# IDLabMedia/image-lens-reproject

Measured on AMD Instinct MI355X. Metric: Mpix/s reprojected (4K RGBA float, bicubic), higher is better.
Workload: dtype f32; 1 GPU; fisheye_to_rect_bicubic: 4096x4096x4 f32 -> 4096x4096x4, eqd->rect, interp=2, num_samples=1; frames_per_launch=16, parallelism=image-sharded x1 (static blocks of the sorted list), no collective

## Files before the change

### image-lens-reproject_amd/csrc/lrp_win_kernel.h

```cpp
#pragma once

#include "lrp_kernel_common.h"
#include "lrp_corner_fill.h"
#include "lrp_tile_kernel.h"
#include "lrp_win_plan.h"
#include "lrp_win_tiers.h"

namespace lrp {

#if defined(LRP_WAVE_STAMPS)
__device__ unsigned long long g_wave_stamps[3 * 65536];
#endif
#if defined(LRP_TIER_STATS)
__device__ unsigned g_tier_stats[8];
#endif


template <int OutLens, int InMode, int QMode, int CH, bool Frames = false, bool GeoRead = false, bool SS = false>
#ifndef LRP_WIN_MINWAVES5
#define LRP_WIN_MINWAVES5 3
#endif
#ifndef LRP_WIN_MINWAVES_AXIS
#define LRP_WIN_MINWAVES_AXIS 4
#endif
#ifndef LRP_WIN_MINWAVES_RAYS
#define LRP_WIN_MINWAVES_RAYS 3
#endif
#ifndef LRP_WIN_MINWAVES_FRAMES
#define LRP_WIN_MINWAVES_FRAMES 4
#endif
#ifndef LRP_WIN_CAP_BIG
#define LRP_WIN_CAP_BIG 1120
#endif
#ifndef LRP_WIN_CAP_BIG5
#define LRP_WIN_CAP_BIG5 1200
#endif
#ifndef LRP_WIN_MINWAVES_BIG
#define LRP_WIN_MINWAVES_BIG 2
#endif
__global__ __launch_bounds__(kWinThreads, (GeoRead && OutLens == kEquirect) ? LRP_WIN_MINWAVES_BIG : CH == 5 ? LRP_WIN_MINWAVES5 : (QMode == 4 ? LRP_WIN_MINWAVES_RAYS : (Frames ? LRP_WIN_MINWAVES_FRAMES : (QMode >= 2 ? LRP_WIN_MINWAVES_AXIS : LRP_WIN_MINWAVES)))) void reproject_bicubic_win_kernel(const KParams Pk) {
  constexpr bool Quad = QMode != 0;
  constexpr bool MirX = QMode == 1 || QMode == 3 || QMode == 4, MirY = QMode == 1 || QMode == 2 || QMode == 4;
  constexpr bool kSharedRays = QMode == 4;
  static_assert(QMode != 4 || OutLens == kEquidistant, "shared rays: the equidistant target");
  constexpr int kAllMirrors = (MirX ? 1 : 0) | (MirY ? 2 : 0);
  using WinBlock = WinBlockT<Quad>;
  static_assert(CH == 3 || CH == 4 || CH == 5, "window kernel: RGB, RGBA or RGBAZ");
  static_assert(!SS || (QMode == 0 && !Frames), "supersampling: plain blocks, no frame loop");
  constexpr int kBlockRows = SS ? 4 : kBlkH;
  static_assert(QMode != 2 || (OutLens != kEquidistant && InMode != kInEquidistant), "rows-only mirroring goes through the column-separable source x");
  static_assert(QMode != 3 || OutLens == kRect, "columns-only mirroring needs vz == -1");
  static_assert(!GeoRead || (QMode == 0 && (OutLens == kRect || (OutLens == kEquirect && !Frames))),
                "GeoRead: plain blocks, one instantiation per source mode (+ the big-window variants)");
  constexpr bool kBigWin = GeoRead && OutLens == kEquirect;
  constexpr int kCap = kBigWin ? (CH == 5 ? LRP_WIN_CAP_BIG5 : LRP_WIN_CAP_BIG) : kWinCap;
#ifndef LRP_BIG_PASSCOLS
#define LRP_BIG_PASSCOLS 64
#endif
  constexpr int kMaxPassCols = kBigWin ? LRP_BIG_PASSCOLS : 64;
  constexpr bool kGeoWrite = !GeoRead && !Frames && QMode == 0 && kWinWaves == 1;
  const bool geo_write = kGeoWrite && (Pk.geo_mode == 1 || Pk.geo_mode == 3) && blockIdx.y == 0;
  const int frames_per_wave = Frames ? (Pk.frames_per_wave > 0 ? Pk.frames_per_wave : 1) : 1;
  const int frame0 = Pk.batch_n > 0 ? (int)blockIdx.y * frames_per_wave : 0;
  const int n_frames = (Frames && Pk.batch_n > 0) ? min(frames_per_wave, Pk.batch_n - frame0) : 1;
  auto frame_src = [&](int f) { return Pk.batch_n > 0 ? Pk.batch_src[frame0 + f] : Pk.src; };
  auto frame_dst = [&](int f) { return Pk.batch_n > 0 ? Pk.batch_dst[frame0 + f] : Pk.dst; };
  KParams P = Pk;
  P.src = frame_src(0);
  P.dst = frame_dst(0);
  constexpr bool kOneBlock = Frames && GeoRead;
  constexpr bool Loop = (InMode == kInEquirectLoop);
  constexpr bool kEdge = InMode == kInRect;
#ifndef LRP_BIG_MAXCOLS
#define LRP_BIG_MAXCOLS 64
#endif
  constexpr bool kSplit = !Frames && (InMode == kInEquirect || InMode == kInEquirectLoop || (InMode == kInRect && CH == 5) || kBigWin);
  constexpr int kMaxStagedCols = kBigWin ? LRP_BIG_MAXCOLS : 64;
  constexpr bool kPassWin = (kSplit || (GeoRead && OutLens == kEquirect)) && (OutLens == kRect || GeoRead || (InMode == kInRect && CH == 5));
  constexpr bool kCoefHere = !kBigWin;
  constexpr bool kTapDma = kBigWin && kWinWaves == 1;
  constexpr int kOutSlots = (CH == 5 && kTapDma) ? 80 : 0;
  static_assert(!kTapDma || (CH == 5 ? (kCap + kOutSlots) * 16 >= 1024 * 20 : kCap >= 1024), "tap DMA: 16 taps x 64 pixels");
  constexpr bool kTapRotate = CH == 5 || kCap < 1027;
  __shared__ float4 s_win[kWinWaves][kCap + kOutSlots];
#ifndef LRP_BIG_PASS_SLOTS
#define LRP_BIG_PASS_SLOTS 4096
#endif
  constexpr int kPassCap = (kTapDma && LRP_BIG_PASS_SLOTS < kCap) ? LRP_BIG_PASS_SLOTS : kCap;

  constexpr bool kListable = GeoRead && InMode == kInRect;
  auto fill_share = [&]() {
    if constexpr (kListable) {
      const uint32_t per_wave = Pk.geo_fill_per_wave;
      if (per_wave != 0 && blockIdx.x % Pk.geo_fill_stride == 0) {
        const uint32_t total = Pk.geo_n_runs * 16u, s0 = blockIdx.x / Pk.geo_fill_stride * per_wave;
        if (s0 < total)
          for (int f = 0; f < n_frames; ++f) corner_fill_rows<CH, kOneBlock>(Pk, frame_src(f), frame_dst(f), s0, min(s0 + per_wave, total));
      }
    }
  };
  int tx, ty;
  bool listed = false;
  constexpr bool kListRec = kListable && kBigWin;
  int list_rec[7] = {0, 0, 0, 0, 0, 0, 0};
  bool have_list_rec = false;
  if constexpr (kListable) listed = Pk.geo_work != nullptr;
  if (listed) {
    typedef const int32_t __attribute__((address_space(4))) *ScalarI;
    const uintptr_t base = reinterpret_cast<uintptr_t>(Pk.geo_work);
    const uint64_t addr = ((uint64_t)(uint32_t)__builtin_amdgcn_readfirstlane((int)(uint32_t)(base >> 32)) << 32 |
                           (uint32_t)__builtin_amdgcn_readfirstlane((int)(uint32_t)base)) + (uint64_t)blockIdx.x * 8u;
    const ScalarI e = reinterpret_cast<ScalarI>(addr);
    tx = e[0];
    ty = e[1];
    if (kListRec && Pk.geo_work_rec != nullptr) {
      const uintptr_t rbase = reinterpret_cast<uintptr_t>(Pk.geo_work_rec);
      const ScalarI r = reinterpret_cast<ScalarI>(((uint64_t)(uint32_t)__builtin_amdgcn_readfirstlane((int)(uint32_t)(rbase >> 32)) << 32 |
                                                   (uint32_t)__builtin_amdgcn_readfirstlane((int)(uint32_t)rbase)) + (uint64_t)blockIdx.x * 32u);
#pragma unroll
      for (int i = 0; i < 7; ++i) list_rec[i] = r[i];
      have_list_rec = true;
    }
    if (tx < 0) {
      fill_share();
      return;
    }
  } else if (!xcd_tile<kWinXcdBand>(P.tiles_x, P.tiles_y, tx, ty, blockIdx.x)) return;
#if defined(LRP_WAVE_STAMPS)
  const unsigned long long stamp_start = wall_clock64();
#endif
  constexpr bool kAliasPairs = (OutLens == kEquirect || GeoRead) && InMode == kInRect && kWinWaves == 1;
  int g_flip = 0;
  bool g_reverse = false;
  if (kAliasPairs && P.alias_pairs != 0 && !listed) {
    if constexpr (QMode == 1) {
      g_flip = (tx & 1) ? 3 : 0;
      tx = (tx & 1) ? P.tiles_x - 1 - (tx >> 1) : (tx >> 1);
    } else if constexpr (QMode == 2) {
      if ((P.tiles_x & 1) == 0) {
        g_flip = (tx & 1) ? 2 : 0;
        tx = (tx >> 1) + ((tx & 1) ? P.tiles_x >> 1 : 0);
      }
    } else if ((P.tiles_x & 1) == 0) {
      g_reverse = (tx & 1) != 0;
      tx = (tx >> 1) + (g_reverse ? P.tiles_x >> 1 : 0);
      ty = g_reverse ? P.tiles_y - 1 - ty : ty;
    }
  }
  int lane = (int)(threadIdx.x & 63u);
  const int wave = __builtin_amdgcn_readfirstlane((int)(threadIdx.x >> 6));
  const int Gs = kOneBlock ? 1 : P.blocks_per_wave;
  const int G = kOneBlock ? 1 : GeoRead ? min(Gs, (P.y_end - P.y_offset + kBlockRows - 1) / kBlockRows - ty * Gs) : Gs;
  auto block_row = [&](int g) { return kOneBlock ? 0 : (kAliasPairs && g_reverse) ? G - 1 - g : g; };
  auto geo_classes = [&]() { return reinterpret_cast<uint8_t *>(P.geo_box) + geo_class_offset(P.out_w, P.out_h); };
  auto geo_class_index = [&](int g) { return (uint32_t)tx * geo_block_rows(P.out_h) + (uint32_t)(ty * Gs + block_row(g)); };
  auto geo_block = [&](int g) { return (uint32_t)(ty * Gs + block_row(g)) * (uint32_t)P.tiles_x + (uint32_t)tx; };
  constexpr bool quad = Quad;
  const int qw = MirX ? (P.out_w + 1) >> 1 : P.out_w;
  const int qh = MirY ? (P.out_h + 1) >> 1 : P.y_end;
  auto image_of = [&](int g) { return ((QMode == 2 ? 2 * g : g) ^ g_flip) & (QMode == 2 ? kAllMirrors : -1); };
  int prow, pcol;
  win_lane_pixel(lane, prow, pcol);
  const int ss_ns = SS ? Pk.num_samples : 1, ss_n = ss_ns * ss_ns, ss_npx = SS ? 64 / ss_n : kBlkW;
  int ss_x = 0, ss_y = 0;
  bool ss_owner = false;
  if constexpr (SS) {
    const int l = min(lane, ss_npx * ss_n - 1);
    pcol = ss_n == 4 ? l >> 2 : ss_n == 16 ? l >> 4 : (l * 57) >> 9;
    prow = 0;
    const int sub = l - pcol * ss_n;
    ss_x = ss_ns == 2 ? sub >> 1 : ss_ns == 4 ? sub >> 2 : (sub * 11) >> 5;
    ss_y = sub - ss_x * ss_ns;
    ss_owner = sub == ss_n - 1 && lane < ss_npx * ss_n;
  }
  const int x = tx * ((SS ? ss_npx : kBlkW) * kWinWaves) + wave * (SS ? ss_npx : kBlkW) + pcol;
  const int y_lane = P.y_offset + ty * (quad ? kBlkH : kBlockRows * Gs) + prow;
  auto pixel_row = [&](int g, int k) { return y_lane + (quad ? 0 : kBlockRows * block_row(g)) + (SS ? k : kPassRows * k); };
  const int xe = x < qw ? x : qw - 1;
  const int in_w = P.in_w;
  SrcView src = source_view<2, CH>(P);
  auto set_frame = [&](int f) {
    P.src = frame_src(f);
    P.dst = frame_dst(f);
    src = source_view<2, CH>(P);
  };
  float4 *const win0 = s_win[wave];
  constexpr bool kRunsEverywhere = CH == 5 && (OutLens == kEquirect || GeoRead) && InMode == kInRect;
  float *out_lds = nullptr;
  if constexpr (CH == 5 && kOutSlots != 0) {
    out_lds = reinterpret_cast<float *>(win0 + kCap);
  } else if constexpr (CH == 5) {
    __shared__ __attribute__((aligned(16))) float s_out[kWinWaves][320];
    out_lds = s_out[wave];
  }
  ColTerms col{0.0f, 0.0f, 0.0f, 0.0f, 0.0f};
  if constexpr (!GeoRead) col = column_terms<OutLens>(P, xe, ss_x);
  ColTerms col_m = col;
  if constexpr (MirX && !kSharedRays) col_m = column_terms<OutLens>(P, P.out_w - 1 - xe, 0);
  float qa[4] = {0.0f, 0.0f, 0.0f, 0.0f}, qb[4] = {0.0f, 0.0f, 0.0f, 0.0f};
  constexpr bool kInEqr = InMode == kInEquirect || InMode == kInEquirectLoop;
  constexpr bool kEqrByTheta = QMode == 3 && kInEqr;
  float qc[(kEqrByTheta || kSharedRays) ? 4 : 1] = {};
  auto quad_xy = [&](int g, int k, float &sx, float &sy) {
    const bool mx = (g & 1) != 0, my = (g >> 1) != 0;
    if constexpr (kSharedRays) {
      const int yk = y_lane + kPassRows * k;
      const uint32_t sgn_x = (mx && 2 * xe != P.out_w - 1) ? 0x80000000u : 0u;
      const uint32_t sgn_y = (my && 2 * yk != P.out_h - 1) ? 0x80000000u : 0u;
      float u, v;
      ray_to_plane<InMode>(P, u2f(f2u(qa[k]) ^ sgn_x), u2f(f2u(qb[k]) ^ sgn_y), qc[k], u, v);
      plane_to_texel<OutLens, InMode>(P, col, u, v, sx, sy);
    } else if constexpr (kEqrByTheta) {
      sx = mx ? qc[k] : qa[k];
      sy = qb[k];
    } else if constexpr (kInEqr) {
      sx = mx ? col_m.sx : col.sx;
      sy = my ? qb[k] : qa[k];
    } else {
      const uint32_t sgn_x = mx ? 0x80000000u : 0u, sgn_y = my ? 0x80000000u : 0u;
      plane_to_texel<OutLens, InMode>(P, mx ? col_m : col, u2f(f2u(qa[k]) ^ sgn_x), u2f(f2u(qb[k]) ^ sgn_y), sx, sy);
    }
  };

  const WinPlanLimits plan_limits = win_plan_limits(P);
  auto slots_of_rows = [](int pitch, int rows) { return win_slots_of_rows<CH>(pitch, rows); };
  auto raw_slots = [&](const WinBlock &b) { return win_raw_slots<CH, kSplit>(b); };
  auto plan_window = [&](WinBlock &b, int w_lo_x, int w_hi_x, int w_lo_ya, int w_hi_ya, int w_lo_yb, int w_hi_yb, bool exact_x, bool exact_y) {
    win_plan_block<CH, Loop, kSplit, kEdge, kCap, kMaxStagedCols>(b, P, plan_limits, w_lo_x, w_hi_x, w_lo_ya, w_hi_ya, w_lo_yb, w_hi_yb, exact_x, exact_y);
  };
  auto clear_block = [](WinBlock &b) { win_clear_block(b); };
  struct Extremes {
// ... 259 lines not shown
      const uint32_t first_row = (uint32_t)__builtin_amdgcn_readfirstlane((int)((uint32_t)b.y_lo * src.row_bytes));
      const uint32_t first_col = (uint32_t)__builtin_amdgcn_readfirstlane((int)((uint32_t)b.x_lo * (4u * CH)));
      const char *first = reinterpret_cast<const char *>(frame) + ((size_t)first_row + (size_t)first_col);
      const uint32_t lds0 = (uint32_t)(uintptr_t)(__attribute__((address_space(3))) void *)win0;
      for (int c0 = 0; c0 < n; c0 += 64) {
        if (c0 + lane < n) {
          const uint32_t lane_bytes = (uint32_t)(c0 + lane) * step;
          const uint32_t lds = lds0 + (uint32_t)c0 * 16u;
          if constexpr (CH == 3)
            asm volatile("s_mov_b32 m0, %0\n\ts_nop 0\n\tglobal_load_lds_dwordx3 %1, %2"
                         :
                         : "s"(__builtin_amdgcn_readfirstlane(lds)), "v"(lane_bytes), "s"(first)
                         : "memory", "m0");
          else
            asm volatile("s_mov_b32 m0, %0\n\ts_nop 0\n\tglobal_load_lds_dwordx4 %1, %2"
                         :
                         : "s"(__builtin_amdgcn_readfirstlane(lds)), "v"(lane_bytes), "s"(first)
                         : "memory", "m0");
          if constexpr (CH == 5) {
            const uint32_t lds_d = lds0 + (uint32_t)n * 16u + (uint32_t)c0 * 4u;
            asm volatile("s_mov_b32 m0, %0\n\ts_nop 0\n\tglobal_load_lds_dword %1, %2"
                         :
                         : "s"(__builtin_amdgcn_readfirstlane(lds_d)), "v"(lane_bytes), "s"(first + 16)
                         : "memory", "m0");
          }
        }
      }
    } else if (b.staged()) {
      float4 *const win = win0;
      asm volatile("s_waitcnt lgkmcnt(0)" ::: "memory");
      const int n_chunks = kMaxPassCols > 64 ? (b.bw + 63) >> 6 : 1;
      for (int chunk = 0; chunk < n_chunks; ++chunk)
      if (chunk * 64 + lane < b.bw) {
        uint32_t lds = (uint32_t)(uintptr_t)(__attribute__((address_space(3))) void *)win + (uint32_t)(b.org() + chunk * 64) * 16u;
        const uint32_t lds_step = (uint32_t)(b.spitch() * 16);
        const uint32_t lane_bytes = (uint32_t)(b.x_lo + chunk * 64 + lane) * (4u * CH);
        const int n_rows = kSplit ? b.rows_of(half) : b.bh;
        if constexpr (kBigWin) {
          const char *const base = reinterpret_cast<const char *>(frame);
          [[maybe_unused]] const char *const base_d = base + 16;
          uint32_t voff = (uint32_t)__builtin_amdgcn_readfirstlane((int)((uint32_t)(kSplit ? b.first_row_of(half) : b.y_lo) * src.row_bytes)) + lane_bytes;
          uint32_t lds_s = (uint32_t)__builtin_amdgcn_readfirstlane((int)lds);
          const uint32_t lds_step_s = (uint32_t)__builtin_amdgcn_readfirstlane((int)lds_step);
          [[maybe_unused]] uint32_t ldsd_s = (uint32_t)__builtin_amdgcn_readfirstlane((int)((uint32_t)(uintptr_t)(__attribute__((address_space(3))) void *)win +
                                                                                       (uint32_t)(b.pitch * n_rows) * 16u + (uint32_t)(chunk * 64) * 4u));
          [[maybe_unused]] const uint32_t ldsd_step = (uint32_t)__builtin_amdgcn_readfirstlane(b.pitch * 4);
          auto request_row = [&]() {
            if constexpr (CH == 4)
              asm volatile("s_mov_b32 m0, %0\n\ts_nop 0\n\tglobal_load_lds_dwordx4 %1, %2" : : "s"(__builtin_amdgcn_readfirstlane((int)lds_s)), "v"(voff), "s"(base) : "memory", "m0");
            else if constexpr (CH == 5) {
              asm volatile("s_mov_b32 m0, %0\n\ts_nop 0\n\tglobal_load_lds_dwordx4 %1, %2" : : "s"(__builtin_amdgcn_readfirstlane((int)lds_s)), "v"(voff), "s"(base) : "memory", "m0");
              asm volatile("s_mov_b32 m0, %0\n\ts_nop 0\n\tglobal_load_lds_dword %1, %2" : : "s"(__builtin_amdgcn_readfirstlane((int)ldsd_s)), "v"(voff), "s"(base_d) : "memory", "m0");
              ldsd_s += ldsd_step;
            } else
              asm volatile("s_mov_b32 m0, %0\n\ts_nop 0\n\tglobal_load_lds_dwordx3 %1, %2" : : "s"(__builtin_amdgcn_readfirstlane((int)lds_s)), "v"(voff), "s"(base) : "memory", "m0");
            lds_s += lds_step_s;
            voff += src.row_bytes;
          };
          int r = 0;
          for (; r + 4 <= n_rows; r += 4) {
            request_row();
            request_row();
            request_row();
            request_row();
          }
          for (; r < n_rows; ++r) request_row();
        } else {
          const char *row = reinterpret_cast<const char *>(frame) + (size_t)(uint32_t)__builtin_amdgcn_readfirstlane((int)((uint32_t)(kSplit ? b.first_row_of(half) : b.y_lo) * src.row_bytes));
          for (int r = 0; r < n_rows; ++r) {
            if constexpr (CH == 4)
              asm volatile("s_mov_b32 m0, %0\n\ts_nop 0\n\tglobal_load_lds_dwordx4 %1, %2"
                           :
                           : "s"(__builtin_amdgcn_readfirstlane(lds)), "v"(lane_bytes), "s"(row)
                           : "memory", "m0");
            else if constexpr (CH == 5) {
              const uint32_t lds_d = (uint32_t)(uintptr_t)(__attribute__((address_space(3))) void *)win +
                                     (uint32_t)(b.pitch * n_rows) * 16u + (uint32_t)(r * b.pitch + chunk * 64) * 4u;
              asm volatile("s_mov_b32 m0, %0\n\ts_nop 0\n\tglobal_load_lds_dwordx4 %1, %2"
                           :
                           : "s"(__builtin_amdgcn_readfirstlane(lds)), "v"(lane_bytes), "s"(row)
                           : "memory", "m0");
              asm volatile("s_mov_b32 m0, %0\n\ts_nop 0\n\tglobal_load_lds_dword %1, %2"
                           :
                           : "s"(__builtin_amdgcn_readfirstlane(lds_d)), "v"(lane_bytes), "s"(row + 16)
                           : "memory", "m0");
            } else
              asm volatile("s_mov_b32 m0, %0\n\ts_nop 0\n\tglobal_load_lds_dwordx3 %1, %2"
                           :
                           : "s"(__builtin_amdgcn_readfirstlane(lds)), "v"(lane_bytes), "s"(row)
                           : "memory", "m0");
            lds += lds_step;
            row += src.row_bytes;
          }
        }
      }
    }
  };

  auto precompute = [&](const WinBlock &b, int h) {
    const int n = b.pitch * b.iyn[h];
    const float4 *const raw = win0 + (b.org() + (b.iy0[h] - 1 - b.y_lo) * b.spitch() + (b.spitch() < 0 ? (b.iyn[h] - 1) * b.spitch() : 0));
    float4 *const planes = win0 + b.c_base;
    auto load4 = [&](int idx, Rgba t[4]) {
      const float4 *q = raw + (idx < n ? idx : n - 1);
      t[0] = as_rgba(q[0]);
      t[1] = as_rgba(q[b.spitch()]);
      t[2] = as_rgba(q[2 * b.spitch()]);
      t[3] = as_rgba(q[3 * b.spitch()]);
    };
    auto emit = [&](int idx, const Rgba t[4]) {
      Rgba inner, m0, cma;
      inner.lo = ((3.0f * (t[1].lo - t[2].lo)) + t[3].lo) - t[0].lo;
      inner.hi = ((3.0f * (t[1].hi - t[2].hi)) + t[3].hi) - t[0].hi;
      m0.lo = (((2.0f * t[0].lo) - (5.0f * t[1].lo)) + (4.0f * t[2].lo)) - t[3].lo;
      m0.hi = (((2.0f * t[0].hi) - (5.0f * t[1].hi)) + (4.0f * t[2].hi)) - t[3].hi;
      cma.lo = t[2].lo - t[0].lo;
      cma.hi = t[2].hi - t[0].hi;
      if (idx < n) {
        planes[idx] = float4{inner.lo.x, inner.lo.y, inner.hi.x, inner.hi.y};
        planes[b.c_plane + idx] = float4{m0.lo.x, m0.lo.y, m0.hi.x, m0.hi.y};
        planes[2 * b.c_plane + idx] = float4{cma.lo.x, cma.lo.y, cma.hi.x, cma.hi.y};
      }
    };
#pragma unroll 1
    for (int i0 = 0; i0 < n; i0 += 128) {
      const bool two = i0 + 64 < n;
      Rgba t0[4], t1[4];
      load4(i0 + lane, t0);
      if (two) load4(i0 + 64 + lane, t1);
      emit(i0 + lane, t0);
      if (two) emit(i0 + 64 + lane, t1);
    }
  };

  auto edge_plane = [&](const WinBlock &b) {
    const float fyc = b.edge() == 2 ? 1.0f : 0.0f, hfyc = 0.5f * fyc;
    float4 *const plane = win0 + b.c_base;
    const float *const raw_d = reinterpret_cast<const float *>(win0 + b.bw);
    float *const plane_d = reinterpret_cast<float *>(plane + b.bw);
#pragma unroll 1
    for (int i0 = 0; i0 < b.bw; i0 += 64) {
      const int i = min(i0 + lane, b.bw - 1);
      const Rgba t = as_rgba(win0[i]);
      const Rgba k = cubic4(t, t, t, t, fyc, hfyc);
      plane[i] = float4{k.lo.x, k.lo.y, k.hi.x, k.hi.y};
      if constexpr (CH == 5) {
        const float dz = raw_d[i];
        plane_d[i] = catmull_rom(dz, dz, dz, dz, fyc, hfyc);
      }
    }
  };

  WinBlock cur, nxt;
  if constexpr (GeoRead) {
    const int cls0 = geo_class(0);
    if (cls0 == 0) geo_fetch(0, cur);
    geo_plan(cur, cls0, 0);
    if constexpr (kOneBlock) {
      auto uniform = [](int &v) { v = __builtin_amdgcn_readfirstlane(v); };
      for (int *v : {&cur.x_lo, &cur.y_lo, &cur.bw, &cur.bh, &cur.pitch, &cur.tier, &cur.iy0[0], &cur.iy0[1], &cur.iyn[0], &cur.iyn[1],
                     &cur.c_plane, &cur.c_base, &cur.tap_base})
        uniform(*v);
    }
  } else {
    coords(0, cur);
  }
  issue(P.src, cur);
  int g_loop = 0, f_loop = 0;
  bool dma_early = false;
  auto issue_next = [&]() {
    if (kOneBlock || f_loop + 1 < n_frames)
      issue(frame_src(f_loop + 1), cur);
    else
      issue(frame_src(0), nxt);
  };
  auto has_next = [&]() { return f_loop + 1 < n_frames || (!kOneBlock && g_loop + 1 < G); };
  auto next_window = [&]() {
    const bool planes_live = (kCoefHere && cur.coef()) || (kEdge && cur.edge() != 0 && cur.edge() < 3);
    dma_early = has_next() && (kOneBlock || !planes_live || f_loop + 1 < n_frames || raw_slots(nxt) <= cur.c_base);
    if (dma_early) issue_next();
  };
  auto accumulate = [&](const Rgba &s) {
    Rgba a4 = px_zero<4>();
    px_add<4>(a4, s);
    if constexpr (CH == 5) a4.e = 0.0f + s.e;
    return Px<CH>{a4.lo, CH >= 4 ? a4.hi : f2{0.0f, 0.0f}, CH == 3 ? a4.hi.x : a4.e};
  };
  struct PassOut {
    int xo, yo, row_step;
    uint32_t first;
    bool whole, mxo;
  };
  auto pass_out = [&](int g, int k) {
    int y_base = y_lane;
    asm volatile("" : "+v"(y_base));
    const int yk = y_base + (quad ? 0 : kBlockRows * block_row(g)) + (SS ? k : kPassRows * k);
    const int yc = yk < qh ? yk : qh - 1;
    const int gm = image_of(g);
    PassOut o;
    o.xo = (quad && (gm & 1)) ? P.out_w - 1 - xe : xe;
    o.yo = (quad && (gm >> 1)) ? P.out_h - 1 - yc : yc;
    const int x_blk = tx * (kBlkW * kWinWaves) + wave * kBlkW;
    const int y_top = P.y_offset + ty * (quad ? kBlkH : kBlockRows * Gs) + (quad ? 0 : kBlockRows * block_row(g)) + (SS ? k : kPassRows * k);
    o.whole = x_blk + kBlkW <= qw && y_top + kPassRows <= qh;
    o.mxo = quad && (gm & 1);
    const bool myo = quad && (gm >> 1);
    o.first = (uint32_t)(myo ? P.out_h - 1 - y_top : y_top) * (uint32_t)P.out_w + (uint32_t)(o.mxo ? P.out_w - x_blk - kBlkW : x_blk);
    o.row_step = myo ? -P.out_w : P.out_w;
    return o;
  };
  auto ss_inside = [&](int g, int k) { return x < qw && pixel_row(g, k) < qh; };
  auto emit = [&](int g, int k, const Rgba &s, auto as_runs, bool runs_rt = true) {
    if constexpr (SS) {
      const Px<CH> sp{s.lo, CH >= 4 ? s.hi : f2{0.0f, 0.0f}, CH == 3 ? s.hi.x : s.e};
      const Px<CH> a = ss_ordered_sum<CH>(sp, (ss_x | ss_y) == 0, ss_n);
      if (ss_owner && ss_inside(g, k)) {
        const PassOut o = pass_out(g, k);
        store_px<CH, false>(P, (uint32_t)o.yo * (uint32_t)P.out_w + (uint32_t)o.xo, a);
      }
      return;
    }
    const Px<CH> a = accumulate(s);
    const PassOut o = pass_out(g, k);
    if constexpr (CH == 5) {
     if constexpr (decltype(as_runs)::value) {
      if (runs_rt && o.whole) {
        float c[5];
        finish_px<5, true>(P, a, c);
        store_rgbaz_run<4>(P, out_lds, prow * kBlkW + (o.mxo ? kBlkW - 1 - pcol : pcol), o.first, o.row_step, c);
        return;
      }
     }
    }
    store_px<CH, true>(P, (uint32_t)o.yo * (uint32_t)P.out_w + (uint32_t)o.xo, a);
  };
  auto emit_corner = [&](int g, const Rgba &s, auto before_last) {
    Px<CH> a = accumulate(s);
    float c[5];
    if constexpr (SS) {
#pragma unroll 1
      for (int t = 1; t < ss_n; ++t) px_add<CH>(a, Px<CH>{s.lo, CH >= 4 ? s.hi : f2{0.0f, 0.0f}, CH == 3 ? s.hi.x : s.e});
      finish_px<CH, false>(P, a, c);
#pragma unroll
      for (int k = 0; k < 4; ++k) {
        if (k == 3) before_last();
        if (ss_owner && ss_inside(g, k)) {
          const PassOut o = pass_out(g, k);
          store_texel_nt<CH>(P.dst + (size_t)((uint32_t)o.yo * (uint32_t)P.out_w + (uint32_t)o.xo) * CH, c);
        }
      }
      return;
    }
    finish_px<CH, true>(P, a, c);
    typedef float v4f_a4 __attribute__((ext_vector_type(4), aligned(4)));
    v4f_a4 q0{0.0f, 0.0f, 0.0f, 0.0f}, q1{0.0f, 0.0f, 0.0f, 0.0f};
    int chunk_row = 0, chunk_col = 0;
    if constexpr (CH == 5) {
      chunk_row = (lane * 3277) >> 16;
      chunk_col = lane - 20 * chunk_row;
      auto pattern = [&](int chunk) {
        const int m = (4 * chunk) % 5;
        auto at = [&](int i) { const int j = (m + i) % 5; return j == 0 ? c[0] : j == 1 ? c[1] : j == 2 ? c[2] : j == 3 ? c[3] : c[4]; };
        return v4f_a4{at(0), at(1), at(2), at(3)};
      };
      q0 = pattern(chunk_col);
      q1 = pattern(4 + lane);
    }
#pragma unroll
    for (int k = 0; k < 4; ++k) {
      if (k == 3) before_last();
      const PassOut o = pass_out(g, k);
      if constexpr (CH == 5) {
        if (o.whole) {
          float *const row0 = P.dst + (size_t)o.first * 5;
          const ptrdiff_t step = (ptrdiff_t)o.row_step * 5;
          __builtin_nontemporal_store(q0, reinterpret_cast<v4f_a4 *>(row0 + chunk_row * step + 4 * chunk_col));
          if (lane < 16) __builtin_nontemporal_store(q1, reinterpret_cast<v4f_a4 *>(row0 + 3 * step + 16 + 4 * lane));
          continue;
        }
      }
      store_texel_nt<CH>(P.dst + (size_t)((uint32_t)o.yo * (uint32_t)P.out_w + (uint32_t)o.xo) * CH, c);
    }
  };
  auto window_sample = [&](const WinBlock &w, float psx, float psy, bool last_pass) -> Rgba {
    const float tx_ = __builtin_truncf(psx), ty_ = __builtin_truncf(psy);
    const int slot0 = __mul24((int)ty_ - 1 - w.y_lo, w.pitch) + ((int)tx_ - 1 - w.x_lo);
    return win_tier_raw<CH>(win0 + slot0, w.pitch, reinterpret_cast<const float *>(win0 + w.pitch * w.bh) + slot0, psx - tx_, psy - ty_, [&]() {
      if (last_pass) next_window();
    });
  };
  auto pass_too_wide = [&](float psx) -> bool {
    const float xa = u2f((uint32_t)__builtin_amdgcn_readlane((int)f2u(psx), 0));
    const float xb = u2f((uint32_t)__builtin_amdgcn_readlane((int)f2u(psx), kBlkW - 1));
    return __builtin_fabsf(xb - xa) >= (float)(kMaxPassCols - 3);
  };
  auto plan_pass_window = [&](WinBlock &w, int lo_x, int hi_x, int lo_y, int hi_y) -> bool {
    if (kBigWin && pass_too_wide(u2f((uint32_t)lo_x))) return false;
    int d0 = 0, d1 = 0;
    wave_box(lo_x, hi_x, lo_y, hi_y, d0, d1);
    clear_block(w);
    w.x_lo = __builtin_amdgcn_readfirstlane((int)u2f((uint32_t)lo_x)) - 1;
    w.y_lo = __builtin_amdgcn_readfirstlane((int)u2f((uint32_t)lo_y)) - 1;
    w.bw = __builtin_amdgcn_readfirstlane((int)u2f((uint32_t)hi_x)) + 2 - w.x_lo + 1;
    w.bh = __builtin_amdgcn_readfirstlane((int)u2f((uint32_t)hi_y)) + 2 - w.y_lo + 1;
    w.pitch = w.bw | 1;
    if (w.bw > kMaxPassCols || slots_of_rows(w.pitch, w.bh) > kPassCap) return false;
    w.tier = 1;
    return true;
  };
  auto pass_window = [&](float psx, float psy, Rgba &s, bool last_pass) -> bool {
    if (!all_interior(psx, psy, 1.0f, src.x_hi, src.y_hi, 2.0f)) return false;
    WinBlock w;
    if (!plan_pass_window(w, (int)f2u(psx), (int)f2u(psx), (int)f2u(psy), (int)f2u(psy))) return false;
    issue(P.src, w);
    asm volatile("s_waitcnt vmcnt(0)" ::: "memory");
    s = window_sample(w, psx, psy, last_pass);
    return true;
  };
  struct PassWin {
    int x_lo, y_lo, bw, bh, pitch;
  };
  const uint32_t pass_lds0 = (uint32_t)__builtin_amdgcn_readfirstlane((int)(uint32_t)(uintptr_t)(__attribute__((address_space(3))) void *)win0);
  auto plan_pass = [&](PassWin &w, float psx, float psy) -> bool {
    if (pass_too_wide(psx)) return false;
    int lo_x = (int)f2u(psx), hi_x = lo_x, lo_y = (int)f2u(psy), hi_y = lo_y, d0 = 0, d1 = 0;
    wave_box(lo_x, hi_x, lo_y, hi_y, d0, d1);
    w.x_lo = __builtin_amdgcn_readfirstlane((int)u2f((uint32_t)lo_x)) - 1;
    w.y_lo = __builtin_amdgcn_readfirstlane((int)u2f((uint32_t)lo_y)) - 1;
    w.bw = __builtin_amdgcn_readfirstlane((int)u2f((uint32_t)hi_x)) + 2 - w.x_lo + 1;
    w.bh = __builtin_amdgcn_readfirstlane((int)u2f((uint32_t)hi_y)) + 2 - w.y_lo + 1;
    w.pitch = w.bw | 1;
    return w.bw <= kMaxPassCols && slots_of_rows(w.pitch, w.bh) <= kPassCap;
  };
  auto request_pass = [&](const PassWin &w) {
    const int n_chunks = (w.bw + 63) >> 6;
    for (int chunk = 0; chunk < n_chunks; ++chunk)
      if (chunk * 64 + lane < w.bw) {
        const uint32_t lane_bytes = (uint32_t)(w.x_lo + chunk * 64 + lane) * (4u * CH);
        const char *row = reinterpret_cast<const char *>(P.src) + (size_t)(uint32_t)__builtin_amdgcn_readfirstlane((int)((uint32_t)w.y_lo * src.row_bytes));
        uint32_t lds = pass_lds0 + (uint32_t)(chunk * 64) * 16u, lds_d = pass_lds0 + (uint32_t)(w.pitch * w.bh) * 16u + (uint32_t)(chunk * 64) * 4u;
        for (int r = 0; r < w.bh; ++r) {
          if constexpr (CH == 3)
            asm volatile("s_mov_b32 m0, %0\n\ts_nop 0\n\tglobal_load_lds_dwordx3 %1, %2" : : "s"(lds), "v"(lane_bytes), "s"(row) : "memory", "m0");
          else
            asm volatile("s_mov_b32 m0, %0\n\ts_nop 0\n\tglobal_load_lds_dwordx4 %1, %2" : : "s"(lds), "v"(lane_bytes), "s"(row) : "memory", "m0");
          if constexpr (CH == 5)
            asm volatile("s_mov_b32 m0, %0\n\ts_nop 0\n\tglobal_load_lds_dword %1, %2" : : "s"(lds_d), "v"(lane_bytes), "s"(row + 16) : "memory", "m0");
          row += src.row_bytes;
          lds += (uint32_t)w.pitch * 16u;
          lds_d += (uint32_t)w.pitch * 4u;
        }
      }
  };
  auto request_taps = [&](float psx, float psy) {
    constexpr uint32_t depth_at = 1024u * 16u;
    const float tx_ = __builtin_truncf(psx), ty_ = __builtin_truncf(psy);
    constexpr uint32_t T = 4u * CH;
    const uint32_t v0 = __umul24((uint32_t)((int)ty_ - 1), src.row_bytes) + (uint32_t)((int)tx_ - 1) * T;
    const char *const base = reinterpret_cast<const char *>(P.src);
    const int j = lane & 3;
#pragma unroll
    for (int t = 0; t < 4; ++t) {
      int got;
      if (t == 0) got = __builtin_amdgcn_mov_dpp((int)v0, 0x00, 0xF, 0xF, false);
      else if (t == 1) got = __builtin_amdgcn_mov_dpp((int)v0, 0x55, 0xF, 0xF, false);
      else if (t == 2) got = __builtin_amdgcn_mov_dpp((int)v0, 0xAA, 0xF, 0xF, false);
      else got = __builtin_amdgcn_mov_dpp((int)v0, 0xFF, 0xF, 0xF, false);
      if constexpr (kTapRotate) {
        if (t == 1) got = __builtin_amdgcn_mov_dpp(got, 0x120 + 4, 0xF, 0xF, false);
        else if (t == 2) got = __builtin_amdgcn_mov_dpp(got, 0x120 + 8, 0xF, 0xF, false);
        else if (t == 3) got = __builtin_amdgcn_mov_dpp(got, 0x120 + 12, 0xF, 0xF, false);
      }
      const uint32_t vt = (uint32_t)got + (uint32_t)j * T;
      {
        const uint32_t o0 = vt, o1 = vt + src.row_bytes, o2 = vt + 2u * src.row_bytes, o3 = vt + 3u * src.row_bytes;
        const uint32_t lds = pass_lds0 + (uint32_t)((4 * t * 64 + (kTapRotate ? 0 : t)) * 16);
        if constexpr (CH == 3)
          asm volatile("s_mov_b32 m0, %0\n\ts_nop 0\n\tglobal_load_lds_dwordx3 %1, %5\n\tglobal_load_lds_dwordx3 %2, %6 offset:1024\n\t"
                       "global_load_lds_dwordx3 %3, %7 offset:2048\n\tglobal_load_lds_dwordx3 %4, %8 offset:3072"
                       :
                       : "s"(lds), "v"(o0), "v"(o1), "v"(o2), "v"(o3), "s"(base), "s"(base - 1024), "s"(base - 2048), "s"(base - 3072)
                       : "memory", "m0");
        else
          asm volatile("s_mov_b32 m0, %0\n\ts_nop 0\n\tglobal_load_lds_dwordx4 %1, %5\n\tglobal_load_lds_dwordx4 %2, %6 offset:1024\n\t"
                       "global_load_lds_dwordx4 %3, %7 offset:2048\n\tglobal_load_lds_dwordx4 %4, %8 offset:3072"
                       :
                       : "s"(lds), "v"(o0), "v"(o1), "v"(o2), "v"(o3), "s"(base), "s"(base - 1024), "s"(base - 2048), "s"(base - 3072)
                       : "memory", "m0");
        if constexpr (CH == 5) {
          const uint32_t lds_d = pass_lds0 + depth_at + (uint32_t)(4 * t * 64 * 4);
          asm volatile("s_mov_b32 m0, %0\n\ts_nop 0\n\tglobal_load_lds_dword %1, %5\n\tglobal_load_lds_dword %2, %6 offset:256\n\t"
                       "global_load_lds_dword %3, %7 offset:512\n\tglobal_load_lds_dword %4, %8 offset:768"
                       :
                       : "s"(lds_d), "v"(o0), "v"(o1), "v"(o2), "v"(o3), "s"(base + 16), "s"(base + 16 - 256), "s"(base + 16 - 512), "s"(base + 16 - 768)
                       : "memory", "m0");
        }
      }
    }
  };
  auto prepare_pass = [&](PassWin &w, float psx, float psy) -> int {
    if (!all_interior(psx, psy, 1.0f, src.x_hi, src.y_hi, 2.0f)) return 0;
    const bool fits = kPassWin && P.win_split != 0 && plan_pass(w, psx, psy);
    if (!fits && !(kTapDma && P.win_tapdma != 0)) return 0;
    asm volatile("s_waitcnt lgkmcnt(0)" ::: "memory");
    if (fits) {
      request_pass(w);
      return 1;
    }
    request_taps(psx, psy);
    return 2;
  };
#pragma unroll 1
  for (int g = 0; g < G; ++g) {
   g_loop = g;
   if constexpr (!GeoRead)
     if ((!Quad || kSharedRays) && !kOneBlock && g + 1 < G) coords(g + 1, nxt);
#pragma unroll 1
   for (int f = 0; f < n_frames; ++f) {
    f_loop = f;
    if constexpr (kOneBlock) asm volatile("" : "+v"(lane));
    if (n_frames > 1 || g == 0) set_frame(f);
    const bool last_frame = f + 1 == n_frames;
    if ((g == 0 && f == 0) || !dma_early || geo_write || SS)
      asm volatile("s_waitcnt vmcnt(0)" ::: "memory");
    else
      asm volatile("s_waitcnt vmcnt(1)" ::: "memory");
    if constexpr (GeoRead)
      if (!kOneBlock && g + 1 < G && f == 0 && geo_class(g + 1) == 0) geo_fetch(g + 1, nxt);
    const float4 *const win = win0;
    const int tier = __builtin_amdgcn_readfirstlane(cur.tier);
    const bool t_coef = kCoefHere && (tier & 2) != 0, t_staged = (tier & 1) != 0, t_whole = (tier & 4) != 0;
    const int t_edge = kEdge ? ((tier >> 6) & 7) : 0;
    const bool t_split = kSplit && (tier & 512) != 0;
#if defined(LRP_TIER_STATS)
    if (lane == 0) atomicAdd(&g_tier_stats[((tier >> 3) & 7) != 0 ? 3 : (tier & 512) != 0 ? 6 : ((tier >> 6) & 7) != 0 ? (((tier >> 6) & 7) < 3 ? 4 : 5) : (kWinCoef && (tier & 2)) ? 0 : (tier & 1) ? 1 : 2], 1u);
#endif
    if (((tier >> 3) & 7) != 0) {
      const Rgba cs = corner_value(cur);
      if (Quad && !kSharedRays && last_frame && !kOneBlock && g + 1 < G) coords(g + 1, nxt);
      if constexpr (GeoRead)
        if (!kOneBlock && g + 1 < G && last_frame) geo_plan(nxt, geo_class(g + 1), g + 1);
      emit_corner(g, cs, [&]() { next_window(); });
      if (!dma_early && has_next()) issue_next();
      if (!kOneBlock && last_frame) cur = nxt;
      continue;
    }
    constexpr bool kRolledUnstaged = kBigWin;
    if constexpr (kRolledUnstaged) {
      if (!t_staged && !t_coef && t_edge == 0) {
        float x0 = cur.sx[0], x1 = cur.sx[1], x2 = cur.sx[2], x3 = cur.sx[3], y0 = cur.sy[0], y1 = cur.sy[1], y2 = cur.sy[2], y3 = cur.sy[3];
        asm volatile("" : "+v"(x0), "+v"(x1), "+v"(x2), "+v"(x3), "+v"(y0), "+v"(y1), "+v"(y2), "+v"(y3));
        auto pass_x = [&](int k) { return k == 0 ? x0 : k == 1 ? x1 : k == 2 ? x2 : x3; };
        auto pass_y = [&](int k) { return k == 0 ? y0 : k == 1 ? y1 : k == 2 ? y2 : y3; };
        constexpr bool kPipeline = kOutSlots == 0;
        PassWin w;
        int kind = 0;
        bool behind_store = true;
#pragma unroll 1
        for (int k = 0; k < 4; ++k) {
          if (k == 3 && !kOneBlock && g + 1 < G && last_frame) geo_plan(nxt, geo_class(g + 1), g + 1);
          const float psx = pass_x(k), psy = pass_y(k);
          if constexpr (!kPipeline) {
            const bool last_pass = k == 3;
            Rgba s;
            if (kPassWin && P.win_split != 0 && pass_window(psx, psy, s, last_pass)) {
            } else if (kTapDma && P.win_tapdma != 0 && all_interior(psx, psy, 1.0f, src.x_hi, src.y_hi, 2.0f)) {
              asm volatile("s_waitcnt lgkmcnt(0)" ::: "memory");
              request_taps(psx, psy);
              asm volatile("s_waitcnt vmcnt(0)" ::: "memory");
              const int j = lane & 3;
              const int slot0 = kTapRotate ? (256 * j + (lane & 48) + ((((lane >> 2) + j) & 3) << 2)) : (257 * j + (lane & ~3));
              s = win_tier_raw<CH, true>(win0 + slot0, 64, reinterpret_cast<const float *>(win0 + 1024) + slot0, psx - __builtin_truncf(psx), psy - __builtin_truncf(psy), [&]() {
                if (last_pass) next_window();
              });
            } else {
              if (last_pass) next_window();
              if constexpr (CH == 5) {
                const Px<5> s5 = sample_direct<2, Loop, 5, LRP_WIN_MINWAVES5 >= 4>(P, src, psx, psy);
                s = Rgba{s5.lo, s5.hi, s5.e};
              } else {
                s = sample_direct<2, Loop, 4, (LRP_WIN_MINWAVES >= 5), 4 * CH>(P, src, psx, psy);
              }
            }
            emit(g, k, s, std::integral_constant<bool, kRunsEverywhere>{}, !GeoRead || P.rgbaz_runs != 0);
            continue;
          }
          if (k == 0) {
            kind = prepare_pass(w, psx, psy);
            behind_store = true;
          }
          const float tx_ = __builtin_truncf(psx), ty_ = __builtin_truncf(psy);
          int next_kind = 0;
          PassWin wn = w;
          auto after_reads = [&]() {
            if (k == 3)
              next_window();
            else if (kPipeline)
              next_kind = prepare_pass(wn, pass_x(k + 1), pass_y(k + 1));
          };
          Rgba s;
          if (kind != 0) {
            if (behind_store)
              asm volatile("s_waitcnt vmcnt(0)" ::: "memory");
            else
              asm volatile("s_waitcnt vmcnt(1)" ::: "memory");
            if (kind == 1) {
              const int slot0 = __mul24((int)ty_ - 1 - w.y_lo, w.pitch) + ((int)tx_ - 1 - w.x_lo);
              s = win_tier_raw<CH>(win0 + slot0, w.pitch, reinterpret_cast<const float *>(win0 + w.pitch * w.bh) + slot0, psx - tx_, psy - ty_, after_reads);
            } else {
              const int j = lane & 3;
              const int slot0 = kTapRotate ? (256 * j + (lane & 48) + ((((lane >> 2) + j) & 3) << 2)) : (257 * j + (lane & ~3));
              s = win_tier_raw<CH, true>(win0 + slot0, 64, reinterpret_cast<const float *>(win0 + 1024) + slot0, psx - tx_, psy - ty_, after_reads);
            }
          } else {
            after_reads();
            if constexpr (CH == 5) {
              const Px<5> s5 = sample_direct<2, Loop, 5, LRP_WIN_MINWAVES5 >= 4>(P, src, psx, psy);
              s = Rgba{s5.lo, s5.hi, s5.e};
            } else {
              s = sample_direct<2, Loop, 4, (LRP_WIN_MINWAVES >= 5), 4 * CH>(P, src, psx, psy);
            }
          }
          emit(g, k, s, std::integral_constant<bool, kRunsEverywhere>{}, !GeoRead || P.rgbaz_runs != 0);
          if constexpr (kPipeline) {
            behind_store = false;
            kind = next_kind;
            w = wn;
          }
        }
        if (!dma_early && has_next()) issue_next();
        if (!kOneBlock && last_frame) cur = nxt;
        continue;
      }
    }
    if (t_edge == 1 || t_edge == 2) edge_plane(cur);
#pragma unroll 2
    for (int h = 0; h < 2; ++h) {
      if (t_coef && (h == 0 || !t_whole)) precompute(cur, h);
      float hx0 = cur.sx[2 * h], hx1 = cur.sx[2 * h + 1], hy0 = cur.sy[2 * h], hy1 = cur.sy[2 * h + 1];
      if constexpr (kBigWin && CH == 5) asm volatile("" : "+v"(hx0), "+v"(hx1), "+v"(hy0), "+v"(hy1));
#pragma unroll(kBigWin && CH == 5 ? 1 : 2)
      for (int kk = 0; kk < 2; ++kk) {
        const int k = 2 * h + kk;
        if (Quad && !kSharedRays && k == 3 && last_frame && !kOneBlock && g + 1 < G) coords(g + 1, nxt);
        if constexpr (GeoRead)
          if (k == 3 && !kOneBlock && g + 1 < G && last_frame) geo_plan(nxt, geo_class(g + 1), g + 1);
        const bool last_pass = k == 3;
        float psx = kk == 0 ? hx0 : hx1, psy = kk == 0 ? hy0 : hy1;
        if constexpr (Quad && !kSharedRays) quad_xy(image_of(g), k, psx, psy);
        asm volatile("" : "+v"(psx), "+v"(psy));
        Rgba s;
        auto after_reads = [&]() {
          if (last_pass) next_window();
          if (t_split && k == 1) issue(P.src, cur, 1);
        };
        if (t_edge != 0) {
          if (t_edge < 3) {
            const float tx_ = __builtin_truncf(psx);
            const int slot = (int)tx_ - 1 - cur.x_lo;
            s = win_tier_edge_row<CH>(win + cur.c_base + slot, reinterpret_cast<const float *>(win + cur.c_base + cur.bw) + slot, psx - tx_, after_reads);
          } else {
            const float ty_ = __builtin_truncf(psy);
            const int slot = (int)ty_ - 1 - cur.y_lo;
            s = win_tier_edge_col<CH>(win + slot, reinterpret_cast<const float *>(win + cur.bh) + slot, psy - ty_, t_edge == 4 ? 1.0f : 0.0f, after_reads);
          }
        } else if (t_coef) {
          const float tx_ = __builtin_truncf(psx), ty_ = __builtin_truncf(psy);
          const int tap = __mul24((int)ty_, cur.spitch()) + (int)tx_ + cur.tap_base;
          s = win_tier_coef<CH>(win + tap, win + (tap + cur.c_delta(h)), cur.c_plane, cur.pitch,
                                reinterpret_cast<const float *>(win + cur.pitch * cur.bh) + (tap - cur.spitch()), psx - tx_, psy - ty_, after_reads);
        } else if (t_staged) {
          const int half = (t_split && h == 1) ? 1 : 0;
          if (t_split && k == 2) {
            if constexpr (SS)
              asm volatile("s_waitcnt vmcnt(0)" ::: "memory");
            else
              asm volatile("s_waitcnt vmcnt(1)" ::: "memory");
          }
          const float tx_ = __builtin_truncf(psx), ty_ = __builtin_truncf(psy);
          const int slot0 = cur.org() + __mul24((int)ty_ - 1 - (kSplit ? cur.first_row_of(half) : cur.y_lo), cur.spitch()) + ((int)tx_ - 1 - cur.x_lo);
          s = win_tier_raw<CH>(win + slot0, cur.spitch(),
                               reinterpret_cast<const float *>(win + cur.pitch * (kSplit ? cur.rows_of(half) : cur.bh)) + slot0, psx - tx_, psy - ty_, after_reads);
        } else if (kRolledUnstaged) {
          __builtin_unreachable();
        } else if (kPassWin && P.win_split != 0 && pass_window(psx, psy, s, last_pass)) {
        } else {
          if (last_pass) next_window();
          if constexpr (CH == 5) {
            const Px<5> s5 = sample_direct<2, Loop, 5, LRP_WIN_MINWAVES5 >= 4>(P, src, psx, psy);
            s = Rgba{s5.lo, s5.hi, s5.e};
          } else {
            s = sample_direct<2, Loop, 4, (LRP_WIN_MINWAVES >= 5), 4 * CH>(P, src, psx, psy);
          }
        }
        emit(g, k, s, std::integral_constant<bool, kRunsEverywhere>{}, !GeoRead || P.rgbaz_runs != 0);
      }
    }
    if (!dma_early && has_next()) issue_next();
    if (!kOneBlock && last_frame) cur = nxt;
   }
  }
  fill_share();
#if defined(LRP_WAVE_STAMPS)
  if (blockIdx.y == 0 && blockIdx.x < 65536u && (threadIdx.x & 63u) == 0) {
    const unsigned hw_id = __builtin_amdgcn_s_getreg((31 << 11) | 4), xcc_id = __builtin_amdgcn_s_getreg((31 << 11) | 20);
    g_wave_stamps[3 * blockIdx.x] = stamp_start;
    g_wave_stamps[3 * blockIdx.x + 1] = wall_clock64();
    g_wave_stamps[3 * blockIdx.x + 2] = (unsigned long long)hw_id | ((unsigned long long)(xcc_id & 15u) << 32) | ((unsigned long long)(unsigned)G << 40) | ((unsigned long long)(blockIdx.x % 8) << 60);
  }
#endif
}

template <int QMode, int CH, bool Frames, bool SS, CellSet Set> struct WinCell {
  template <int OutLens, int InMode> static constexpr TileKernelFn kernel() {
    if constexpr (in_cell_set(Set, OutLens, InMode) && mirror_cell(QMode, OutLens, InMode) && (!Frames || frame_loop_cell(OutLens, InMode)))
      return reproject_bicubic_win_kernel<OutLens, InMode, QMode, CH, Frames, false, SS>;
    else
      return nullptr;
  }
};
template <int CH, bool Frames, bool SS, CellSet Set> struct WinGeoCell {
  template <int OutLens, int InMode> static constexpr TileKernelFn kernel() {
    if constexpr (in_cell_set(Set, OutLens, InMode) && (geo_read_cell(OutLens, InMode) || (!Frames && !SS && geo_big_cell(OutLens, InMode))))
      return reproject_bicubic_win_kernel<OutLens, InMode, 0, CH, Frames, true, SS>;
    else
      return nullptr;
  }
};

template <int QMode, int CH, bool GeoRead, bool SS, CellSet Set> TileKernelFn win_kernel(const KParams &P, int out_lens, int in_mode) {
  if constexpr (GeoRead) {
    const int im = geo_read_in_mode(in_mode);
    if constexpr (SS)
      return cell_kernel<WinGeoCell<CH, false, true, Set>>(kRect, im);
    else if (P.frames_per_wave > 1)
      return cell_kernel<WinGeoCell<CH, true, false, Set>>(kRect, im);
    else
      return cell_kernel<WinGeoCell<CH, false, false, Set>>((P.big_windows != 0 && geo_big_cell(kEquirect, im)) ? kEquirect : kRect, im);
  } else if constexpr (SS) {
    return cell_kernel<WinCell<0, CH, false, true, Set>>(out_lens, in_mode);
  } else {
    return P.frames_per_wave > 1 ? cell_kernel<WinCell<QMode, CH, true, false, Set>>(out_lens, in_mode)
                                 : cell_kernel<WinCell<QMode, CH, false, false, Set>>(out_lens, in_mode);
  }
}

template <int QMode, int CH, bool GeoRead = false, bool SS = false, CellSet Set = kStdCells>
inline hipError_t launch_win_bicubic_impl(KParams P, int out_lens, int in_mode, hipStream_t stream) {
  static_assert(!GeoRead || QMode == 0, "the geometry cache feeds plain blocks");
  static_assert(!SS || QMode == 0, "supersampling: plain blocks");
  if (GeoRead && (P.geo_mode != 2 || P.y_offset != 0 || P.y_end != P.out_h)) return hipErrorInvalidValue;
  if ((SS ? (P.num_samples < 2 || P.num_samples > 4) : P.num_samples != 1) || (SS && !GeoRead && P.geo_mode != 0 && P.geo_mode != 1)) return hipErrorInvalidValue;
  constexpr int kRowsPerBlock = SS ? kPassRows : kBlkH;
  const int rows = P.y_end - P.y_offset;
  if (QMode != 0) {
    const int qw = (QMode == 1 || QMode == 3 || QMode == 4) ? (P.out_w + 1) / 2 : P.out_w;
    const int qh = (QMode == 1 || QMode == 2 || QMode == 4) ? (P.out_h + 1) / 2 : P.out_h;
    P.tiles_x = (qw + kBlkW * kWinWaves - 1) / (kBlkW * kWinWaves);
    P.tiles_y = (qh + kBlkH - 1) / kBlkH;
    P.blocks_per_wave = (QMode == 1 || QMode == 4) ? 4 : 2;
  } else {
    const int cols_per_block = SS ? 64 / (P.num_samples * P.num_samples) : kBlkW;
    P.tiles_x = (P.out_w + cols_per_block * kWinWaves - 1) / (cols_per_block * kWinWaves);
    const int row_blocks = (rows + kRowsPerBlock - 1) / kRowsPerBlock;
#ifndef LRP_SS_STRIP
#define LRP_SS_STRIP 4
#endif
    int G = SS ? LRP_SS_STRIP : LRP_WIN_STRIP;
    if (GeoRead && !SS && P.blocks_per_wave > 0) G = std::min(P.blocks_per_wave, kGeoStripRows);
    if (P.batch_n > 1 && !(out_lens == kEquirect && in_mode == kInRect)) G = 1;
    const bool strip_forced = GeoRead && !SS && P.blocks_per_wave > 0;
    if (GeoRead && !SS && !strip_forced && in_mode == kInRect && P.big_windows == 0 && P.batch_n <= 1) G = 1;
    const long long min_waves = GeoRead ? 16384 : 8192;
    while (!strip_forced && G > 1 && (long long)P.tiles_x * kWinWaves * ((row_blocks + G - 1) / G) < min_waves) G >>= 1;
    if (GeoRead && P.geo_work != nullptr && in_mode != kInRect) return hipErrorInvalidValue;
    if (GeoRead && P.geo_work != nullptr) G = 1;
    P.blocks_per_wave = G;
    P.tiles_y = (row_blocks + G - 1) / G;
  }
  int n_tiles = P.tiles_x * P.tiles_y;
  if (n_tiles <= 0) return hipSuccess;
  int groups = P.batch_n > 0 ? P.batch_n : 1;
  const int frames_override = P.frames_per_wave;
  P.frames_per_wave = 1;
  if (P.batch_n > 1) {
    const long long units = (long long)n_tiles * kWinWaves * P.batch_n;
    int F = (int)std::min<long long>(P.batch_n, std::max<long long>(1, units / 8192));
    if (out_lens == kEquirect && in_mode == kInRect) F = 1;
    if (GeoRead && P.big_windows != 0) F = 1;
    if (frames_override > 0) F = std::max(1, std::min(P.batch_n, frames_override));
    if (P.geo_mode == 1 || P.geo_mode == 3) F = 1;
    if (SS) F = 1;
    P.frames_per_wave = F;
    if (F > 1 && !win_kernel<QMode, CH, GeoRead, SS, Set>(P, out_lens, in_mode)) P.frames_per_wave = F = 1;
    if (GeoRead && F > 1 && P.blocks_per_wave != 1) {
      P.blocks_per_wave = 1;
      P.tiles_y = (rows + kRowsPerBlock - 1) / kRowsPerBlock;
      n_tiles = P.tiles_x * P.tiles_y;
    }
    groups = (P.batch_n + F - 1) / F;
  }
  const TileKernelFn fn = win_kernel<QMode, CH, GeoRead, SS, Set>(P, out_lens, in_mode);
  if (!fn) return hipErrorInvalidValue;
  unsigned grid_x = (unsigned)(kXcds * xcd_rows(P.tiles_y, kWinXcdBand) * P.tiles_x);
  if (GeoRead && P.geo_work != nullptr) {
    if (kWinWaves != 1) return hipErrorInvalidValue;
    if (P.geo_n_work == 0) return hipSuccess;
    grid_x = P.geo_n_work;
  }
// ... 6 lines not shown
```

Before: 180,000 Mpix/s.

## Hoist per-pass LDS tap addresses and output offsets out of the frame loop

In the one-block multi-frame GeoRead path, the per-pass fractional coordinates, LDS tap byte addresses and (for RGBA) destination byte offsets are computed once before the frame loop and kept in registers. Each frame iteration then reads window taps and stores outputs through these fixed offsets. The aim is to drop the repeated trunc, slot and address arithmetic and the per-pixel output index math for every frame. The cost is extra VGPRs held across the loop, which can lower occupancy, plus a duplicated tier-dispatch body.

```diff
diff --git a/image-lens-reproject_amd/csrc/lrp_win_kernel.h b/image-lens-reproject_amd/csrc/lrp_win_kernel.h
--- a/image-lens-reproject_amd/csrc/lrp_win_kernel.h
+++ b/image-lens-reproject_amd/csrc/lrp_win_kernel.h
@@ -15,6 +15,12 @@
 __device__ unsigned g_tier_stats[8];
 #endif
 
+constexpr int frame_loop_hoist(int in_mode, int ch) {
+  return (ch == 5 || (in_mode == kInRect && ch == 3)) ? 1 : 2;
+}
+template <class T> __device__ __forceinline__ const T *lds_ptr(uint32_t byte_addr) {
+  return static_cast<const T *>(__builtin_assume_aligned((const T *)(__attribute__((address_space(3))) const T *)(uintptr_t)byte_addr, sizeof(T)));
+}
 
 template <int OutLens, int InMode, int QMode, int CH, bool Frames = false, bool GeoRead = false, bool SS = false>
 #ifndef LRP_WIN_MINWAVES5
@@ -69,6 +75,7 @@
   P.src = frame_src(0);
   P.dst = frame_dst(0);
   constexpr bool kOneBlock = Frames && GeoRead;
+  constexpr int kHoist = kOneBlock ? frame_loop_hoist(InMode, CH) : 0;
   constexpr bool Loop = (InMode == kInEquirectLoop);
   constexpr bool kEdge = InMode == kInRect;
 #ifndef LRP_BIG_MAXCOLS
@@ -77,6 +84,8 @@
   constexpr bool kSplit = !Frames && (InMode == kInEquirect || InMode == kInEquirectLoop || (InMode == kInRect && CH == 5) || kBigWin);
   constexpr int kMaxStagedCols = kBigWin ? LRP_BIG_MAXCOLS : 64;
   constexpr bool kPassWin = (kSplit || (GeoRead && OutLens == kEquirect)) && (OutLens == kRect || GeoRead || (InMode == kInRect && CH == 5));
+  static_assert(kHoist == 0 || (!kSplit && !kPassWin && !kBigWin && !SS && QMode == 0),
+                "the held-state pass bodies have no split half, no pass window, no rolled loop, no mirror image");
   constexpr bool kCoefHere = !kBigWin;
   constexpr bool kTapDma = kBigWin && kWinWaves == 1;
   constexpr int kOutSlots = (CH == 5 && kTapDma) ? 80 : 0;
@@ -642,6 +651,12 @@
   };
 
   WinBlock cur, nxt;
+  struct PassLane {
+    float a, b;
+    uint32_t addr, dst;
+  };
+  PassLane pl[4] = {};
+  size_t blk_dst_bytes = 0;
   if constexpr (GeoRead) {
     const int cls0 = geo_class(0);
     if (cls0 == 0) geo_fetch(0, cur);
@@ -683,7 +698,7 @@
   };
   auto pass_out = [&](int g, int k) {
     int y_base = y_lane;
-    asm volatile("" : "+v"(y_base));
+    if constexpr (kHoist < 2) asm volatile("" : "+v"(y_base));
     const int yk = y_base + (quad ? 0 : kBlockRows * block_row(g)) + (SS ? k : kPassRows * k);
     const int yc = yk < qh ? yk : qh - 1;
     const int gm = image_of(g);
@@ -699,6 +714,7 @@
     o.row_step = myo ? -P.out_w : P.out_w;
     return o;
   };
+  auto pass_dst = [&](int k) { return reinterpret_cast<float *>(reinterpret_cast<char *>(P.dst) + blk_dst_bytes + (size_t)pl[k].dst); };
   auto ss_inside = [&](int g, int k) { return x < qw && pixel_row(g, k) < qh; };
   auto emit = [&](int g, int k, const Rgba &s, auto as_runs, bool runs_rt = true) {
     if constexpr (SS) {
@@ -722,7 +738,13 @@
       }
      }
     }
-    store_px<CH, true>(P, (uint32_t)o.yo * (uint32_t)P.out_w + (uint32_t)o.xo, a);
+    if constexpr (kHoist >= 2) {
+      float c[5];
+      finish_px<CH, true>(P, a, c);
+      store_texel_nt<CH>(pass_dst(k), c);
+    } else {
+      store_px<CH, true>(P, (uint32_t)o.yo * (uint32_t)P.out_w + (uint32_t)o.xo, a);
+    }
   };
   auto emit_corner = [&](int g, const Rgba &s, auto before_last) {
     Px<CH> a = accumulate(s);
@@ -769,7 +791,10 @@
           continue;
         }
       }
-      store_texel_nt<CH>(P.dst + (size_t)((uint32_t)o.yo * (uint32_t)P.out_w + (uint32_t)o.xo) * CH, c);
+      if constexpr (kHoist >= 2)
+        store_texel_nt<CH>(pass_dst(k), c);
+      else
+        store_texel_nt<CH>(P.dst + (size_t)((uint32_t)o.yo * (uint32_t)P.out_w + (uint32_t)o.xo) * CH, c);
     }
   };
   auto window_sample = [&](const WinBlock &w, float psx, float psy, bool last_pass) -> Rgba {
@@ -900,6 +925,36 @@
     request_taps(psx, psy);
     return 2;
   };
+  const uint32_t lds0 = (uint32_t)(uintptr_t)(__attribute__((address_space(3))) void *)win0;
+  if constexpr (kHoist >= 1) {
+    const int tier = cur.tier;
+    const int edge = kEdge ? ((tier >> 6) & 7) : 0;
+    const int x_blk = tx * (kBlkW * kWinWaves) + wave * kBlkW, y_blk = P.y_offset + ty * kBlockRows;
+    if constexpr (kHoist >= 2) blk_dst_bytes = (size_t)((uint32_t)y_blk * (uint32_t)P.out_w + (uint32_t)x_blk) * (4u * CH);
+#pragma unroll
+    for (int k = 0; k < 4; ++k) {
+      const float psx = cur.sx[k], psy = cur.sy[k];
+      const float tx_ = __builtin_truncf(psx), ty_ = __builtin_truncf(psy);
+      int slot = 0;
+      pl[k].a = psx - tx_;
+      pl[k].b = psy - ty_;
+      if (edge != 0) {
+        slot = edge < 3 ? cur.c_base + ((int)tx_ - 1 - cur.x_lo) : (int)ty_ - 1 - cur.y_lo;
+      } else if (kCoefHere && (tier & 2) != 0) {
+        slot = __mul24((int)ty_, cur.spitch()) + (int)tx_ + cur.tap_base;
+      } else if ((tier & 1) != 0) {
+        slot = cur.org() + __mul24((int)ty_ - 1 - cur.y_lo, cur.spitch()) + ((int)tx_ - 1 - cur.x_lo);
+      } else {
+        pl[k].a = psx;
+        pl[k].b = psy;
+      }
+      pl[k].addr = lds0 + (uint32_t)slot * 16u;
+      if constexpr (kHoist >= 2) {
+        const PassOut o = pass_out(0, k);
+        pl[k].dst = (uint32_t)((o.yo - y_blk) * P.out_w + (o.xo - x_blk)) * (4u * CH);
+      }
+    }
+  }
 #pragma unroll 1
   for (int g = 0; g < G; ++g) {
    g_loop = g;
@@ -918,7 +973,8 @@
     if constexpr (GeoRead)
       if (!kOneBlock && g + 1 < G && f == 0 && geo_class(g + 1) == 0) geo_fetch(g + 1, nxt);
     const float4 *const win = win0;
-    const int tier = __builtin_amdgcn_readfirstlane(cur.tier);
+    int tier = __builtin_amdgcn_readfirstlane(cur.tier);
+    if constexpr (kHoist >= 1) asm volatile("" : "+s"(tier));
     const bool t_coef = kCoefHere && (tier & 2) != 0, t_staged = (tier & 1) != 0, t_whole = (tier & 4) != 0;
     const int t_edge = kEdge ? ((tier >> 6) & 7) : 0;
     const bool t_split = kSplit && (tier & 512) != 0;
@@ -1027,7 +1083,8 @@
 #pragma unroll 2
     for (int h = 0; h < 2; ++h) {
       if (t_coef && (h == 0 || !t_whole)) precompute(cur, h);
-      float hx0 = cur.sx[2 * h], hx1 = cur.sx[2 * h + 1], hy0 = cur.sy[2 * h], hy1 = cur.sy[2 * h + 1];
+      float hx0 = 0.0f, hx1 = 0.0f, hy0 = 0.0f, hy1 = 0.0f;
+      if constexpr (kHoist == 0) hx0 = cur.sx[2 * h], hx1 = cur.sx[2 * h + 1], hy0 = cur.sy[2 * h], hy1 = cur.sy[2 * h + 1];
       if constexpr (kBigWin && CH == 5) asm volatile("" : "+v"(hx0), "+v"(hx1), "+v"(hy0), "+v"(hy1));
 #pragma unroll(kBigWin && CH == 5 ? 1 : 2)
       for (int kk = 0; kk < 2; ++kk) {
@@ -1038,13 +1095,38 @@
         const bool last_pass = k == 3;
         float psx = kk == 0 ? hx0 : hx1, psy = kk == 0 ? hy0 : hy1;
         if constexpr (Quad && !kSharedRays) quad_xy(image_of(g), k, psx, psy);
-        asm volatile("" : "+v"(psx), "+v"(psy));
+        if constexpr (kHoist == 0) asm volatile("" : "+v"(psx), "+v"(psy));
         Rgba s;
         auto after_reads = [&]() {
           if (last_pass) next_window();
           if (t_split && k == 1) issue(P.src, cur, 1);
         };
-        if (t_edge != 0) {
+        if constexpr (kHoist >= 1) {
+          asm volatile("" : "+v"(pl[k].a), "+v"(pl[k].b), "+v"(pl[k].addr));
+          if constexpr (kHoist >= 2) asm volatile("" : "+v"(pl[k].dst));
+          const PassLane q = pl[k];
+          auto depth_at = [&](int plane_bytes) { return lds_ptr<float>((q.addr >> 2) + (lds0 - (lds0 >> 2)) + (uint32_t)plane_bytes); };
+          if (t_edge != 0) {
+            if (t_edge < 3)
+              s = win_tier_edge_row<CH>(lds_ptr<float4>(q.addr), depth_at((cur.c_base + cur.bw) * 16 - cur.c_base * 4), q.a, after_reads);
+            else
+              s = win_tier_edge_col<CH>(lds_ptr<float4>(q.addr), depth_at(cur.bh * 16), q.b, t_edge == 4 ? 1.0f : 0.0f, after_reads);
+          } else if (t_coef) {
+            s = win_tier_coef<CH>(lds_ptr<float4>(q.addr), lds_ptr<float4>(q.addr + (uint32_t)(cur.c_delta(h) * 16)), cur.c_plane, cur.pitch,
+                                  depth_at(cur.pitch * cur.bh * 16 - cur.spitch() * 4), q.a, q.b, after_reads);
+          } else if (t_staged) {
+            s = win_tier_raw<CH>(lds_ptr<float4>(q.addr), cur.spitch(), depth_at(cur.pitch * cur.bh * 16), q.a, q.b, after_reads);
+          } else {
+            if (last_pass) next_window();
+            const float gx = q.a, gy = q.b;
+            if constexpr (CH == 5) {
+              const Px<5> s5 = sample_direct<2, Loop, 5, LRP_WIN_MINWAVES5 >= 4>(P, src, gx, gy);
+              s = Rgba{s5.lo, s5.hi, s5.e};
+            } else {
+              s = sample_direct<2, Loop, 4, (LRP_WIN_MINWAVES >= 5), 4 * CH>(P, src, gx, gy);
+            }
+          }
+        } else if (t_edge != 0) {
           if (t_edge < 3) {
             const float tx_ = __builtin_truncf(psx);
             const int slot = (int)tx_ - 1 - cur.x_lo;
```

Result: faster. 185,800 Mpix/s, median of 6 (+3.3%).
